# rdd0582/mri_superresolution

Hardware: AMD Instinct MI355X
Metric: 2D MRI slices/sec (train fwd+bwd) 256×256 U-Net; PSNR/SSIM vs ref (higher is better)
Workload: dtype bf16; 1 GPU; UNetSuperRes base_filters=64 depth=4, 256x256 slices -> 512x512, batch=16/GPU bf16, L1+SSIM(0.4), train step fwd+bwd+Adam+SSIM metric; global_batch=16, parallelism=dp1

## Files before the change

### include/mrisr.h

```cpp
#ifndef MRISR_H
#define MRISR_H

#include <stddef.h>
#include <stdint.h>

#ifdef __cplusplus
extern "C" {
#endif

#define MRISR_OK 0
#define MRISR_E_ARG (-1)
#define MRISR_E_SHAPE (-2)
#define MRISR_E_DTYPE (-3)
#define MRISR_E_HIP (-4)
#define MRISR_E_UNSUPPORTED (-5)

#define MRISR_F32 0
#define MRISR_BF16 1
#define MRISR_F16 2

#define MRISR_SRC_RAW 0
#define MRISR_SRC_NORM 1
#define MRISR_SRC_RELU 2
#define MRISR_SP_NONE 0
#define MRISR_SP_POOL2 1
#define MRISR_SP_UP2 2
#define MRISR_COMBINE_CONCAT 0
#define MRISR_COMBINE_BLEND 1
#ifndef MRISR_STAT_SLOTS
#define MRISR_STAT_SLOTS 16
#endif
#define MRISR_SP_HEAD 3
#define MRISR_OUT_PLAIN 0
#define MRISR_OUT_PIXEL_SHUFFLE2 1

typedef struct {
    const void* ptr;
    const float* scale;
    const float* shift;
    int32_t C, H, W;
    int32_t mode;
    int32_t spatial;
    int32_t off_y, off_x;
} mrisr_src;

typedef struct {
    int32_t dtype;
    int32_t N, H, W;
    int32_t Cin, Cout;
    int32_t ksize;
    int32_t nsrc;
    int32_t combine;
    int32_t out_mode;
    int32_t groups;
    int32_t relu_out;
    mrisr_src src[2];
    const float* blend_alpha;
    const void* wpacked;
    const float* bias;
    void* out;
    double* stats;
    const void* relu_mask;
    int32_t cu_limit;
    int32_t reserved_;
    const void* wpacked_ring;
} mrisr_conv_desc;

const char* mrisr_last_error(void);
int mrisr_version(void);
int mrisr_stat_slots(void);

size_t mrisr_packed_weight_bytes(int dtype, int Cout, int Cin, int ksize);
#define MRISR_PACK_RING 256
#define MRISR_PACK_UPADJ 512
int mrisr_conv_ring_bn(int dtype, int Cout, int Cin, int ksize);
size_t mrisr_packed_weight_bytes_ring(int dtype, int Cout, int Cin, int ksize);
int mrisr_pack_weights(int dtype, const float* w, int Cout, int Cin, int ksize, int transpose_flip,
                       void* packed, void* stream);
typedef struct {
    const float* w;
    void* packed;
    int32_t Cout, Cin, ksize, transpose_flip;
} mrisr_pack_job;
int mrisr_pack_weights_batched(int dtype, const mrisr_pack_job* jobs_device, int njobs, void* stream);
int mrisr_conv_forward(const mrisr_conv_desc* d, void* stream);
int mrisr_conv_variant(const mrisr_conv_desc* d, int wgrad, char* out, size_t n);
int mrisr_conv_wgrad(const mrisr_conv_desc* d, const void* dy, float* dw, float* workspace, size_t workspace_floats,
                     void* stream);
size_t mrisr_conv_wgrad_workspace_floats(const mrisr_conv_desc* d);

size_t mrisr_packed_weight_bytes_upadj(int dtype, int Cout, int Cin, int ksize);
int mrisr_conv_upadj(const mrisr_conv_desc* d, const void* g, void* d_low, void* stream);

int mrisr_stem_forward(int dtype, const float* x, const float* w, void* out, double* stats,
                       int N, int H, int W, int Cout, int groups, void* stream);
int mrisr_stem_wgrad(int dtype, const float* x, const void* dy, float* dw,
                     int N, int H, int W, int Cout, void* stream);
int mrisr_stem_forward_multi(int dtype, const float* x, const float* w, void* out, double* stats,
                             int N, int H, int W, int Cin, int Cout, int groups, void* stream);
int mrisr_stem_wgrad_multi(int dtype, const float* x, const void* dy, float* dw,
                           int N, int H, int W, int Cin, int Cout, void* stream);

int mrisr_gn_finalize(const double* stats, const float* gamma, const float* beta, float* scale,
                      float* shift, float* meanrstd, int N, int C, int groups, double count,
                      float eps, void* stream);

int mrisr_norm_pool2(int dtype, const void* x, const float* scale, const float* shift, void* out, int N,
                     int H, int W, int C, void* stream);
// ... 221 lines not shown
```

### mri_superresolution_amd/_lib.py

```python
from __future__ import annotations

import ctypes as C
import os

from .tuning import TUNING

_HERE = os.path.dirname(os.path.abspath(__file__))
LIB_PATH = TUNING.lib_path or os.path.join(_HERE, "libmrisr.so")

F32, BF16, F16 = 0, 1, 2
SRC_RAW, SRC_NORM, SRC_RELU = 0, 1, 2
SP_NONE, SP_POOL2, SP_UP2, SP_HEAD = 0, 1, 2, 3
COMBINE_CONCAT, COMBINE_BLEND = 0, 1
OUT_PLAIN, OUT_PIXEL_SHUFFLE2 = 0, 1
UP2_BILINEAR, UP2_BICUBIC, UP2_SHARP_BILINEAR = 0, 1, 2
WINDOW_F32, WINDOW_I16 = 0, 1
VOLBLEND_SET, VOLBLEND_ADD, VOLBLEND_FINISH = 0, 1, 2
MORPH_DILATE, MORPH_ERODE = 0, 1
RESAMPLE_LINEAR, RESAMPLE_CUBIC, RESAMPLE_AREA, RESAMPLE_LANCZOS4 = 1, 2, 3, 4
PACK_RING = 256
PACK_UPADJ = 512
STAT_SLOTS = 16

_vp, _fp, _dp, _i, _f, _d, _sz = C.c_void_p, C.c_void_p, C.c_void_p, C.c_int, C.c_float, C.c_double, C.c_size_t


class Src(C.Structure):
    _fields_ = [("ptr", _vp), ("scale", _fp), ("shift", _fp), ("C", C.c_int32), ("H", C.c_int32),
                ("W", C.c_int32), ("mode", C.c_int32), ("spatial", C.c_int32), ("off_y", C.c_int32),
                ("off_x", C.c_int32)]


class ConvDesc(C.Structure):
    _fields_ = [("dtype", C.c_int32), ("N", C.c_int32), ("H", C.c_int32), ("W", C.c_int32),
                ("Cin", C.c_int32), ("Cout", C.c_int32), ("ksize", C.c_int32), ("nsrc", C.c_int32),
                ("combine", C.c_int32), ("out_mode", C.c_int32), ("groups", C.c_int32),
                ("relu_out", C.c_int32), ("src", Src * 2), ("blend_alpha", _fp), ("wpacked", _vp),
                ("bias", _fp), ("out", _vp), ("stats", _dp), ("relu_mask", _vp), ("cu_limit", C.c_int32),
                ("reserved_", C.c_int32), ("wpacked_ring", _vp)]


class PackJob(C.Structure):
    _fields_ = [("w", _fp), ("packed", _vp), ("Cout", C.c_int32), ("Cin", C.c_int32), ("ksize", C.c_int32),
                ("transpose_flip", C.c_int32)]


class AugGeo(C.Structure):
    _fields_ = [("cos_a", C.c_float), ("sin_a", C.c_float), ("rotate", C.c_int32), ("flip", C.c_int32),
                ("fill", C.c_int32), ("brightness", C.c_float)]


class AugPhoto(C.Structure):
    _fields_ = [("contrast", C.c_float), ("mean", C.c_int32), ("noise_sigma", C.c_float), ("seed", C.c_uint32)]


class GnBwdFin(C.Structure):
    _fields_ = [("red", _fp), ("gamma", _fp), ("meanrstd", _fp), ("dgamma", _fp), ("dbeta", _fp),
                ("alpha_slots", _fp), ("alpha", _fp), ("dalpha", _fp), ("count", C.c_double),
                ("alpha_sign", C.c_float), ("groups", C.c_int32)]


class BlendBranch(C.Structure):
    _fields_ = [("x", _vp), ("scale", _fp), ("shift", _fp), ("meanrstd", _fp), ("red", _fp), ("alpha_slots", _fp),
                ("weight_mode", C.c_int32), ("reserved_", C.c_int32)]


class Consumer(C.Structure):
    _fields_ = [("da", _vp), ("C_total", C.c_int32), ("c_off", C.c_int32), ("H", C.c_int32),
                ("W", C.c_int32), ("spatial", C.c_int32), ("off_y", C.c_int32), ("off_x", C.c_int32),
                ("weight_mode", C.c_int32), ("head_out", _fp), ("head_w", _fp), ("head_part", _fp),
                ("head_dw", _fp), ("head_db", _fp)]


SIGNATURES = {
    "mrisr_last_error": (C.c_char_p, []),
    "mrisr_version": (_i, []),
    "mrisr_stat_slots": (_i, []),
    "mrisr_packed_weight_bytes": (_sz, [_i, _i, _i, _i]),
    "mrisr_conv_ring_bn": (_i, [_i, _i, _i, _i]),
    "mrisr_packed_weight_bytes_ring": (_sz, [_i, _i, _i, _i]),
    "mrisr_pack_weights": (_i, [_i, _fp, _i, _i, _i, _i, _vp, _vp]),
    "mrisr_pack_weights_batched": (_i, [_i, _vp, _i, _vp]),
    "mrisr_conv_forward": (_i, [C.POINTER(ConvDesc), _vp]),
    "mrisr_packed_weight_bytes_upadj": (_sz, [_i, _i, _i, _i]),
    "mrisr_conv_upadj": (_i, [C.POINTER(ConvDesc), _vp, _vp, _vp]),
    "mrisr_conv_variant": (_i, [C.POINTER(ConvDesc), _i, C.c_char_p, _sz]),
    "mrisr_conv_wgrad": (_i, [C.POINTER(ConvDesc), _vp, _fp, _fp, _sz, _vp]),
    "mrisr_conv_wgrad_workspace_floats": (_sz, [C.POINTER(ConvDesc)]),
    "mrisr_stem_forward": (_i, [_i, _fp, _fp, _vp, _dp, _i, _i, _i, _i, _i, _vp]),
    "mrisr_stem_wgrad": (_i, [_i, _fp, _vp, _fp, _i, _i, _i, _i, _vp]),
    "mrisr_stem_forward_multi": (_i, [_i, _fp, _fp, _vp, _dp, _i, _i, _i, _i, _i, _i, _vp]),
    "mrisr_stem_wgrad_multi": (_i, [_i, _fp, _vp, _fp, _i, _i, _i, _i, _i, _vp]),
    "mrisr_gn_finalize": (_i, [_dp, _fp, _fp, _fp, _fp, _fp, _i, _i, _i, _d, _f, _vp]),
    "mrisr_norm_pool2": (_i, [_i, _vp, _fp, _fp, _vp, _i, _i, _i, _i, _vp]),
    "mrisr_norm_upsample2": (_i, [_i, _vp, _fp, _fp, _vp, _i, _i, _i, _i, _vp]),
    "mrisr_norm_blend": (_i, [_i, _vp, _fp, _fp, _vp, _fp, _fp, _fp, _vp, _i, _i, _i, _i, _vp]),
    "mrisr_upsample2_stats": (_i, [_i, _vp, _vp, _dp, _i, _i, _i, _i, _i, _vp]),
    "mrisr_upsample2_adjoint": (_i, [_i, _vp, _vp, _i, _i, _i, _i, _vp]),
    "mrisr_act_bwd_reduce": (_i, [_i, _vp, _fp, _fp, _fp, _i, C.POINTER(Consumer), _fp, _vp, _fp, _fp, _i, _i, _i, _i, _i, _vp]),
    "mrisr_act_bwd_finalize": (_i, [_fp, _fp, _fp, _fp, _fp, _fp, _i, _i, _i, _d, _fp, _fp, _fp, _f, _vp]),
    "mrisr_act_bwd_apply": (_i, [_i, _vp, _vp, _fp, _vp, _i, _i, _i, _i, _i, _fp, _vp]),
    "mrisr_act_bwd_apply_fused": (_i, [_i, _vp, _fp, _fp, _i, C.POINTER(Consumer), _fp, _fp, C.POINTER(GnBwdFin), _vp, _i, _i,
                                       _i, _i, _vp]),
    "mrisr_act_bwd_onepass_slots": (_i, []),
    "mrisr_act_bwd_onepass_barrier_words": (_i, []),
    "mrisr_act_bwd_onepass_ok": (_i, [_i, _i, C.POINTER(Consumer), _i, _i, _i, _i]),
# ... 40 lines not shown
    "mrisr_resample_taps": (_i, [_i, _i, _i, _i, _vp, _vp, _fp]),
    "mrisr_f32_resample_letterbox": (_i, [_fp, _i, _i, _i, _vp, _fp, _i, _i, _vp, _fp, _i, _i, _i, _i, _i, _i, _f, _i, _fp, _vp, _vp]),
    "mrisr_f32_percentile_workspace_bytes": (_sz, [_i]),
    "mrisr_f32_percentile_bounds": (_i, [_fp, _sz, _i, _d, _d, _fp, _vp, _vp]),
    "mrisr_f32_window_normalise": (_i, [_fp, _fp, _sz, _i, _fp, _vp]),
    "mrisr_f32_window_restore": (_i, [_fp, _fp, _sz, _i, _i, _vp, _vp]),
    "mrisr_f32_volume_up2_blend": (_i, [_fp, _i, _i, _i, _i, _fp, _i, _i, _i, _vp, _vp]),
    "mrisr_f32_volume_down2": (_i, [_fp, _i, _i, _i, _i, _fp, _vp]),
    "mrisr_f32_volume_up2": (_i, [_fp, _i, _i, _i, _i, _i, _fp, _vp]),
    "mrisr_f32_volume_metrics": (_i, [_fp, _fp, _i, _i, _i, _f, _f, _i, _dp, _vp]),
    "mrisr_volume_metrics_finalize": (_i, [_dp, _i, _i, _i, _f, _dp, _vp]),
    "mrisr_f32_volume_metrics_masked": (_i, [_fp, _fp, _vp, _i, _i, _i, _f, _f, _i, _dp, _vp]),
    "mrisr_volume_metrics_finalize_masked": (_i, [_dp, _i, _i, _i, _f, _dp, _vp]),
    "mrisr_f32_volume_otsu_workspace_bytes": (_sz, []),
    "mrisr_f32_volume_otsu_mask": (_i, [_fp, _i, _i, _i, _vp, _dp, _vp, _vp]),
    "mrisr_u8_volume_morph": (_i, [_vp, _i, _i, _i, _i, _i, _vp, _vp, _vp]),
    "mrisr_u8_volume_label": (_i, [_vp, _i, _i, _i, _i, _i, _i, _vp, _vp]),
    "mrisr_u8_volume_label_workspace_bytes": (_sz, [_i, _i, _i]),
    "mrisr_u8_volume_keep_largest": (_i, [_vp, _i, _i, _i, _i, _vp, _dp, _vp, _vp]),
    "mrisr_u8_volume_fill_holes": (_i, [_vp, _i, _i, _i, _i, _vp, _dp, _vp, _vp]),
}

_lib = None
ABI_VERSION = 314


def load():
    global _lib
    if _lib is not None:
        return _lib
    if not os.path.exists(LIB_PATH):
        raise RuntimeError(
            f"{LIB_PATH} not found: the HIP kernel library is not built. Run "
            "`python -m mri_superresolution_amd.build` (needs hipcc); there is no CPU fallback.")
    lib = C.CDLL(LIB_PATH)
    missing = [name for name in SIGNATURES if not hasattr(lib, name)]
    if missing:
        raise RuntimeError(f"{LIB_PATH} lacks {len(missing)} symbol(s) of include/mrisr.h ({', '.join(missing[:4])}...): "
                           "header/library drift - rebuild with `python -m mri_superresolution_amd.build`")
    for name, (res, args) in SIGNATURES.items():
        fn = getattr(lib, name)
        fn.restype = res
        fn.argtypes = args
    if int(lib.mrisr_version()) != ABI_VERSION:
        raise RuntimeError(f"{LIB_PATH} is version {int(lib.mrisr_version())}, these bindings need {ABI_VERSION} (struct layouts "
                           "changed): rebuild with `python -m mri_superresolution_amd.build`")
    global STAT_SLOTS
# ... 48 lines not shown
```

### mri_superresolution_amd/csrc/api.cpp

```cpp
#include "common.h"
thread_local char g_mrisr_err[512] = "";
extern "C" const char* mrisr_last_error(void) { return g_mrisr_err; }
extern "C" int mrisr_version(void) { return 314; }
extern "C" int mrisr_stat_slots(void) { return MRISR_STAT_SLOTS; }
```

### mri_superresolution_amd/csrc/conv_common.h

```cpp
#pragma once
#include "common.h"

constexpr int kConvThreads = 256;
constexpr int kRowBytes = 64;
constexpr int kMaxHaloIter = 6;

__device__ __forceinline__ int swz(int row) { return (row >> 2) & 3; }
__device__ __forceinline__ int lds_off(int row, int chunk) {
    return row * kRowBytes + ((chunk ^ swz(row)) << 4);
}

constexpr int kHaloRowBytes = 80;
__device__ __forceinline__ int halo_off(int row, int chunk) { return row * kHaloRowBytes + (chunk << 4); }

static inline size_t conv_halo_bytes() { return (size_t)kMaxHaloIter * 64 * kHaloRowBytes; }
constexpr int kDmaHaloRows = 340;
constexpr int kDmaHaloBytes = kDmaHaloRows * 64;
static inline size_t conv_halo_total(bool dma) { return dma ? 4 * (size_t)kDmaHaloBytes : 2 * conv_halo_bytes(); }
static inline bool conv_weights_stationary(int nchunks, size_t wimg, bool dma = false) {
    return nchunks * wimg + conv_halo_total(dma) + (64 + 128) * sizeof(float) <= 159 * 1024;
}
static inline int conv_wgrad_fast(int dtype, int loader, int ks, int tw_log2, int Cout, int Cin) {
    if (dtype == MRISR_F32 || loader != MRISR_SP_NONE || ks != 3 || tw_log2 != 5) return 0;
    const int nfo = Cout % 64 == 0 ? 2 : (Cout <= 32 ? 1 : 0), nfi = Cin % 64 == 0 ? 2 : (Cin <= 32 ? 1 : 0);
// ... 30 lines not shown
    const float* shift;
    int C, H, W, mode, off_y, off_x;
    unsigned img_bytes;
};

struct ConvParams {
    SrcDev src[2];
    const float* blend_alpha;
    const void* wpacked;
    const float* bias;
    void* out;
    double* stats;
    const void* mask;
    const void* dy;
    float* dw;
    float* wsp;
    int N, H, W, Cin, CinP, Cout, CoutP;
    int nsrc, combine, out_mode, groups, relu_out;
    int tw_log2, th, tiles_x, tiles_y, ncb, nchunks;
    int ksplit;
    int ws;
    int ntiles, tiles_per_block;
    int cus;
    int dbg;
};
#ifdef MRISR_TUNING
#define DBG(p) ((p).dbg)
#else
#define DBG(p) 0
#endif

#define PIN_F(q, src, f) { auto v__ = (src).f; asm volatile("" : "+s"(v__)); (q).f = v__; }
__device__ __forceinline__ ConvParams pin_params(const ConvParams& in) {
    ConvParams q = in;
    PIN_F(q, in, H) PIN_F(q, in, W) PIN_F(q, in, Cout) PIN_F(q, in, N) PIN_F(q, in, nchunks) PIN_F(q, in, tw_log2)
    PIN_F(q, in, th) PIN_F(q, in, tiles_x) PIN_F(q, in, tiles_y) PIN_F(q, in, nsrc) PIN_F(q, in, dbg)
    PIN_F(q, in, groups) PIN_F(q, in, relu_out) PIN_F(q, in, out) PIN_F(q, in, stats) PIN_F(q, in, bias)
    PIN_F(q, in, dy) PIN_F(q, in, dw) PIN_F(q, in, wsp) PIN_F(q, in, mask) PIN_F(q, in, Cin) PIN_F(q, in, combine)
    PIN_F(q, in, src[0].ptr) PIN_F(q, in, src[0].scale) PIN_F(q, in, src[0].shift) PIN_F(q, in, src[0].C)
    PIN_F(q, in, src[0].H) PIN_F(q, in, src[0].W) PIN_F(q, in, src[0].mode) PIN_F(q, in, src[0].off_y)
    PIN_F(q, in, src[0].off_x) PIN_F(q, in, src[0].img_bytes)
    PIN_F(q, in, src[1].ptr) PIN_F(q, in, src[1].scale) PIN_F(q, in, src[1].shift) PIN_F(q, in, src[1].C)
    PIN_F(q, in, src[1].H) PIN_F(q, in, src[1].W) PIN_F(q, in, src[1].mode) PIN_F(q, in, src[1].off_y)
    PIN_F(q, in, src[1].off_x) PIN_F(q, in, src[1].img_bytes)
    return q;
}
// ... 258 lines not shown
```

### mri_superresolution_amd/csrc/conv_fwd.hip

```cpp
#include <stdlib.h>
#include <string.h>

#include "conv_common.h"

int num_cus();
int conv_fill_params(const mrisr_conv_desc* d, ConvParams& p, const char* who) {
    if (!d) MRISR_FAIL(MRISR_E_ARG, "%s: null descriptor", who);
    if (!mrisr_dtype_ok(d->dtype)) MRISR_FAIL(MRISR_E_DTYPE, "%s: dtype %d", who, d->dtype);
    if (d->ksize != 1 && d->ksize != 3) MRISR_FAIL(MRISR_E_UNSUPPORTED, "%s: ksize %d", who, d->ksize);
    if (d->nsrc < 1 || d->nsrc > 2) MRISR_FAIL(MRISR_E_ARG, "%s: nsrc %d", who, d->nsrc);
    if (d->N <= 0 || d->H <= 0 || d->W <= 0 || d->Cin <= 0 || d->Cout <= 0)
        MRISR_FAIL(MRISR_E_SHAPE, "%s: bad dims N%d H%d W%d Cin%d Cout%d", who, d->N, d->H, d->W, d->Cin, d->Cout);
    const int vec = mrisr_vec(d->dtype);
    memset(&p, 0, sizeof(p));
    int csum = 0;
    for (int s = 0; s < d->nsrc; ++s) {
        const mrisr_src& a = d->src[s];
        if (!a.ptr) MRISR_FAIL(MRISR_E_ARG, "%s: src%d null", who, s);
        if (a.C % vec) MRISR_FAIL(MRISR_E_SHAPE, "%s: src%d channels %d not a multiple of %d", who, s, a.C, vec);
        if (a.mode == MRISR_SRC_NORM && (!a.scale || !a.shift)) MRISR_FAIL(MRISR_E_ARG, "%s: src%d NORM without scale/shift", who, s);
        if (s > 0 && a.spatial != MRISR_SP_NONE) MRISR_FAIL(MRISR_E_UNSUPPORTED, "%s: spatial transform on src1", who);
        if (d->nsrc > 1 && a.spatial != MRISR_SP_NONE) MRISR_FAIL(MRISR_E_UNSUPPORTED, "%s: spatial transform with 2 sources", who);
        int vh = a.H, vw = a.W;
        if (a.spatial == MRISR_SP_POOL2) { vh = a.H / 2; vw = a.W / 2; }
// ... 84 lines not shown
        bool raw = true;
        for (int i = 0; i < d->nsrc; ++i) raw = raw && d->src[i].mode == MRISR_SRC_RAW;
        snprintf(out, n, "conv_wgrad_rows_kernel<%s,%d,%d,%d>", t, d->Cout % 64 ? 1 : 2, d->Cin % 64 ? 1 : 2, raw ? 1 : 0);
    } else if (wgrad) {
        snprintf(out, n, "conv_wgrad_kernel<%s,%d,%d,%d>", t, loader, d->ksize,
                 conv_wgrad_fast(d->dtype, loader, d->ksize, p.tw_log2, d->Cout, d->Cin));
    } else if (conv_ring_eligible(d, p)) {
        snprintf(out, n, "conv_ring_kernel<%s,2,4>", t);
    } else if (conv_pc_eligible(d, p)) {
        snprintf(out, n, "conv_pc_kernel<%s,%d%s>", t, d->src[0].mode == MRISR_SRC_NORM ? 1 : 0, conv_pc_kind(d, p) == 2 ? ",64" : "");
    } else if (conv1x1_gemm_eligible(d, p)) {
        snprintf(out, n, "conv1x1_gemm_kernel<%s,%d>", t, d->src[0].mode == MRISR_SRC_NORM ? 1 : 0);
    } else {
        const int BN = conv_choose_bn(d->Cout);
        const size_t wimg = (size_t)d->ksize * d->ksize * BN * kRowBytes;
        const bool dma = conv_dma_halo(p, d->src[0].spatial);
        const int ws = conv_weights_stationary(p.nchunks, wimg, dma) ? 1 : 0;
        snprintf(out, n, "conv_igemm_kernel<%s,%d,%d,%d,%d,%d,%d>", t, BN, loader, d->ksize, ws,
                 d->out_mode == MRISR_OUT_PIXEL_SHUFFLE2 ? 1 : (d->relu_mask ? kEpiMask : 0), dma ? 1 : 0);
    }
    return MRISR_OK;
}

extern "C" int mrisr_conv_forward(const mrisr_conv_desc* d, void* stream) {
    ConvParams p;
    int rc = conv_fill_params(d, p, "conv_forward");
    if (rc) return rc;
    if (!d->wpacked || !d->out) MRISR_FAIL(MRISR_E_ARG, "conv_forward: null weights/out");
    if (d->out_mode == MRISR_OUT_PIXEL_SHUFFLE2 && (d->Cout % 16)) MRISR_FAIL(MRISR_E_SHAPE, "conv_forward: pixel shuffle needs Cout%%16==0");
    if (d->relu_mask && (d->out_mode != MRISR_OUT_PLAIN || d->Cout % (mrisr_vec(d->dtype))))
        MRISR_FAIL(MRISR_E_UNSUPPORTED, "conv_forward: relu_mask needs a plain output with Cout a multiple of the 16-byte vector");
    if (d->stats && (d->groups <= 0 || d->Cout % d->groups)) MRISR_FAIL(MRISR_E_SHAPE, "conv_forward: Cout %d not divisible by groups %d", d->Cout, d->groups);
    if (conv_ring_eligible(d, p)) return launch_conv_ring(d, p, (hipStream_t)stream);
    if (conv_pc_eligible(d, p)) return launch_conv_pc(d, p, (hipStream_t)stream);
    if (conv1x1_gemm_eligible(d, p)) return launch_conv1x1_gemm(d, p, (hipStream_t)stream);
    if (d->ksize == 3 && d->W > 16 && d->H >= 16) {
        p.th = 16; p.tw_log2 = 4;
        p.tiles_x = ceil_div(d->W, 16); p.tiles_y = ceil_div(d->H, 16);
    }
    const int sp = d->src[0].spatial;
    hipStream_t s = (hipStream_t)stream;
    const int BN = conv_choose_bn(d->Cout);
    if (d->dtype == MRISR_BF16) return launch_conv_igemm_bf16(p, BN, sp, d->ksize, s);
    if (d->dtype == MRISR_F16) return launch_conv_igemm_f16(p, BN, sp, d->ksize, s);
    return launch_conv_igemm_f32(p, BN, sp, d->ksize, s);
}
```

### mri_superresolution_amd/csrc/conv_igemm.h

```cpp
#pragma once
#include <mutex>
#include <type_traits>

#include "conv_common.h"

template <typename T> struct Mma;
template <> struct Mma<bf16_t> {
    typedef bf16x8 frag;
    static __device__ __forceinline__ f32x16 run(frag a, frag b, f32x16 c) {
        return __builtin_amdgcn_mfma_f32_32x32x16_bf16(a, b, c, 0, 0, 0);
    }
};
template <> struct Mma<f16_t> {
    typedef f16x8 frag;
    static __device__ __forceinline__ f32x16 run(frag a, frag b, f32x16 c) {
        return __builtin_amdgcn_mfma_f32_32x32x16_f16(a, b, c, 0, 0, 0);
    }
};
template <> struct Mma<float> {
    typedef f32x4 frag;
    static __device__ __forceinline__ f32x16 run(frag a, frag b, f32x16 c) {
#pragma unroll
        for (int j = 0; j < 4; ++j) c = __builtin_amdgcn_mfma_f32_32x32x2f32(a[j], b[j], c, 0, 0, 0);
        return c;
// ... 685 lines not shown
                        [&](int st) { pace_dma(plan, st); });
                PT_MARK(6)
                if (it_jj == p.nchunks - 1) {
                    epilogue(it_n, it_ty0, it_tx0);
                    PT_MARK(4)
                    if (p.stats && (!nx_valid || nx_n != it_n)) flush_stats(it_n);
                    PT_MARK(9)
                }
            } else {
#pragma unroll
                for (int st = 0; st < 2 * NTAPS; ++st) pace_dma(plan, st);
            }
            gkc = nx_kc;
            it_jj = nx_jj; it_tile = nx_tile; it_n = nx_n; it_ty0 = nx_ty0; it_tx0 = nx_tx0;
        }
#ifdef MRISR_PHASE_TIMING
        if (blockIdx.x == gridDim.x / 2 && lane == 0) {
            pt_acc[10] = __builtin_amdgcn_s_memrealtime() - pt_r0;
#pragma unroll
            for (int k = 0; k < 12; ++k) atomicAdd(&g_phase_cycles[threadIdx.x >> 6][k], pt_acc[k]);
            if (threadIdx.x == 0) atomicAdd(&g_phase_cycles[0][11], 1ull);
        }
#endif
        return;
    }
    int cur_tile = tile0, cur_kc = 0, cur_n = 0, cur_ty0 = 0, cur_tx0 = 0;
    int nxt_tile = tile0, nxt_kc = 0, nxt_n = 0, nxt_ty0 = 0, nxt_tx0 = 0;
    int ep_n = 0, ep_ty0 = 0, ep_tx0 = 0;
    bool ep_pending = false;
    const int nitems0 = nh0 * p.nchunks;
    if (nitems > 0) {
        decode(cur_tile, cur_n, cur_ty0, cur_tx0);
        set_geom(cur_n, cur_ty0, cur_tx0);
        issue(cur_n, 0, cur_ty0, cur_tx0);
    }
    if constexpr (!WS) {
        if (half == 0 && nitems0 > 0) dma_weights(0, 0, std::integral_constant<int, 4>{});
        __builtin_amdgcn_s_waitcnt(0x0f70);
        if constexpr (NH != 1) __syncthreads();
    }
    if constexpr (NH == 1) {
        if (wave == 0 && nitems > 0) lds_aff[lane] = pf.aff;
        __syncthreads();
    }
    if (__builtin_amdgcn_readfirstlane(threadIdx.x) >= 256) __builtin_amdgcn_s_setprio(1);
    PT_DECL
// ... 40 lines not shown
                ep_pending = true;
                ep_n = cur_n; ep_ty0 = cur_ty0; ep_tx0 = cur_tx0;
            }
            cur_tile = nxt_tile; cur_kc = nxt_kc; cur_n = nxt_n; cur_ty0 = nxt_ty0; cur_tx0 = nxt_tx0;
            if constexpr (NH == 1) {
                if (wave == 0) lds_aff[lane] = pf.aff;
            }
          }
            PT_MARK(6)
        }
        if (!(DBG(p) & 64)) __syncthreads();
#ifdef MRISR_PHASE_TIMING
        if (phase >= 0 && (phase & 1) == 0) PT_MARK(5) else PT_MARK(7)
#endif
    }
#ifdef MRISR_PHASE_TIMING
    if (blockIdx.x == gridDim.x / 2 && lane == 0) {
        pt_acc[10] = __builtin_amdgcn_s_memrealtime() - pt_r0;
#pragma unroll
        for (int k = 0; k < 12; ++k) atomicAdd(&g_phase_cycles[threadIdx.x >> 6][k], pt_acc[k]);
        if (threadIdx.x == 0) atomicAdd(&g_phase_cycles[0][11], 1ull);
    }
#endif
}

#ifdef MRISR_PHASE_TIMING
static int conv_igemm_phase(unsigned long long* out96) {
    unsigned long long v[96] = {};
    if (!out96) return (int)hipMemcpyToSymbol(HIP_SYMBOL(g_phase_cycles), v, sizeof(v));
    const int rc = (int)hipMemcpyFromSymbol(v, HIP_SYMBOL(g_phase_cycles), sizeof(v));
    if (rc) return rc;
    for (int k = 0; k < 96; ++k) out96[k] += v[k];
    return 0;
}
#endif

int launch_gn_stats(int dtype, const void* x, double* stats, int N, int HW, int C, int groups, hipStream_t s);

template <typename T, int BN, int SPATIAL, int KS, bool DMA>
static int launch_conv_v(ConvParams& p, hipStream_t s) {
    const size_t wimg = (size_t)KS * KS * BN * kRowBytes;
    p.ws = conv_weights_stationary(p.nchunks, wimg, DMA) ? 1 : 0;
    const size_t lds = conv_halo_total(DMA) + (p.ws ? p.nchunks : 2) * wimg + (BN + 128) * sizeof(float);
    p.ntiles = p.N * p.tiles_y * p.tiles_x;
    int per_cb = p.cus / p.ncb;
    if (per_cb < 1) per_cb = 1;
// ... 71 lines not shown
```

### mri_superresolution_amd/csrc/norm.hip

```cpp
#include "common.h"

__global__ void gn_finalize_kernel(const double* __restrict__ stats, const float* __restrict__ gamma,
                                   const float* __restrict__ beta, float* __restrict__ scale,
                                   float* __restrict__ shift, float* __restrict__ meanrstd, int N, int C,
                                   int groups, double count, float eps) {
    const int idx = blockIdx.x * blockDim.x + threadIdx.x;
    if (idx >= N * C) return;
    const int n = idx / C, c = idx - n * C;
    const int gs = C / groups, g = c / gs;
    typedef __attribute__((ext_vector_type(2))) double f64x2;
    f64x2 v[MRISR_STAT_SLOTS];
#pragma unroll
    for (int k = 0; k < MRISR_STAT_SLOTS; ++k) v[k] = *reinterpret_cast<const f64x2*>(stats + ((size_t)(k * N + n) * groups + g) * 2);
    double s = 0.0, ss = 0.0;
#pragma unroll
    for (int k = 0; k < MRISR_STAT_SLOTS; ++k) { s += v[k][0]; ss += v[k][1]; }
    const double mean = s / count;
    double var = ss / count - mean * mean;
    if (var < 0) var = 0;
    const float rstd = (float)(1.0 / sqrt(var + (double)eps));
    const float m = (float)mean;
    const float sc = gamma[c] * rstd;
    scale[idx] = sc;
    shift[idx] = beta[c] - m * sc;
    if (c == g * gs) {
        meanrstd[((size_t)n * groups + g) * 2] = m;
        meanrstd[((size_t)n * groups + g) * 2 + 1] = rstd;
    }
}

extern "C" int mrisr_gn_finalize(const double* stats, const float* gamma, const float* beta, float* scale,
                                 float* shift, float* meanrstd, int N, int C, int groups, double count,
                                 float eps, void* stream) {
    if (!stats || !gamma || !beta || !scale || !shift || !meanrstd) MRISR_FAIL(MRISR_E_ARG, "gn_finalize: null pointer");
    if (groups <= 0 || C % groups) MRISR_FAIL(MRISR_E_SHAPE, "gn_finalize: C %d groups %d", C, groups);
    gn_finalize_kernel<<<ceil_div(N * C, 256), 256, 0, (hipStream_t)stream>>>(stats, gamma, beta, scale, shift,
                                                                             meanrstd, N, C, groups, count, eps);
    MRISR_CHECK_LAUNCH("gn_finalize");
    return MRISR_OK;
}

struct ConsumerDev {
    const void* da;
    int C_total, c_off, H, W, spatial, off_y, off_x, weight_mode;
    const float* head_out;
    const float* head_w;
    float* head_part;
    float* head_dw;
    float* head_db;
};
struct ActBwdParams {
// ... 1915 lines not shown
```

### mri_superresolution_amd/engine.py

```python
from __future__ import annotations

import ctypes as C
from dataclasses import dataclass
from typing import Dict, List, Optional, Tuple

import torch

from . import _lib as L
from .launch import GN_GROUPS, Consumer, dgrad_desc, gn_finalize, marshal_consumers
from .tuning import TUNING


def _dt(dtype: torch.dtype) -> int:
    if dtype == torch.bfloat16:
        return L.BF16
    if dtype == torch.float16:
        return L.F16
    if dtype == torch.float32:
        return L.F32
    raise ValueError(f"unsupported compute dtype {dtype} (use torch.float32, torch.float16 or torch.bfloat16)")


@dataclass(frozen=True, eq=False)
class Node:
    name: str
    C: int
    gamma: str
    beta: str
    shuffled: bool = False


@dataclass(frozen=True, eq=False)
# ... 117 lines not shown
        for j in range(1, depth):
            skip, cout = xs[depth - 1 - j], f * 2 ** (depth - 1 - j)
            up = node(f"up{j}.up.1", cout, f"up{j}.up.2.weight", f"up{j}.up.2.bias")
            self.layers.append(Layer(f"up{j}.up.1", 2 * cout, cout, 1, (Source(u),), up, post_up=True))
            u = dconv(f"up{j}.conv", (Source(skip), Source(up)), 2 * cout, cout)
        fb = node("final_up_bilinear.1", f // 2, "final_up_bilinear.2.weight", "final_up_bilinear.2.bias")
        self.layers.append(Layer("final_up_bilinear.1", f, f // 2, 3, (Source(u),), fb, up_src=True))
        ps = node("final_up_pixelshuffle.conv", f // 2, "final_up_pixelshuffle.norm.weight",
                  "final_up_pixelshuffle.norm.bias", shuffled=True)
        self.layers.append(Layer("final_up_pixelshuffle.conv", f, 2 * f, 3, (Source(u),), ps, bias=True,
                                 out_mode=L.OUT_PIXEL_SHUFFLE2))
        fc = node("final_conv.0", f // 2, "final_conv.1.weight", "final_conv.1.bias")
        self.layers.append(Layer("final_conv.0", f // 2, f // 2, 3, (Source(fb), Source(ps)), fc,
                                 combine=L.COMBINE_BLEND, blend_src=True))
        self.head_in = fc
        self._blend_sibling: Dict[Node, Node] = {}
        for layer in self.layers:
            if layer.combine == L.COMBINE_BLEND:
                a, b = (src.node for src in layer.srcs)
                self._blend_sibling[a], self._blend_sibling[b] = b, a
        self._packed: Dict[tuple, torch.Tensor] = {}
        self._packed_token = None
        self.timer: Optional[KernelTimer] = None

    def _launch(self, kind, desc, fn):
        if self.timer is None:
            return fn()
        flops = 2.0 * desc.N * desc.H * desc.W * desc.Cin * desc.Cout * desc.ksize * desc.ksize
        if kind == "upadj":
            flops /= 4
        buf = C.create_string_buffer(96)
        L.call("mrisr_conv_variant", C.byref(desc), {"wgrad": 1, "upadj": 2}.get(kind, 0), buf, 96)
        self.timer.launch(buf.value.decode(), flops, fn)

    def _packed_buf(self, layer: Layer, w, dt: int, flip: int, ring: bool = False, upadj: bool = False):
        key = (layer.name, dt, "upadj") if upadj else (layer.name, dt, flip, "ring") if ring else (layer.name, dt, flip)
        buf = self._packed.get(key)
        if buf is None or buf.device != w.device:
            if upadj:
                nbytes = L.load().mrisr_packed_weight_bytes_upadj(dt, layer.cout, layer.cin, layer.ks)
            else:
                size = L.load().mrisr_packed_weight_bytes_ring if ring else L.load().mrisr_packed_weight_bytes
                nbytes = size(dt, layer.cin if flip else layer.cout, layer.cout if flip else layer.cin, layer.ks)
            buf = torch.empty(nbytes, dtype=torch.uint8, device=w.device)
            self._packed[key] = buf
        return buf
# ... 73 lines not shown
        if s.spatial == L.SP_POOL2:
            return n.H // 2, n.W // 2
        if s.spatial == L.SP_UP2:
            return 2 * n.H, 2 * n.W
        return n.H, n.W

    def forward(self, params, x: torch.Tensor, dtype: torch.dtype, training: bool, weights_token=None):
        dt = _dt(dtype)
        dev = x.device
        N, _, H, W = x.shape
        es = 4 if dtype == torch.float32 else 2
        mins = 2 ** (self.depth - 1)
        if H < mins or W < mins:
            raise ValueError(f"input must be at least {mins}x{mins} ({self.depth - 1} 2x2 max-pools)")
        st = L.stream_ptr()
        f = self.f
        p = _Pass()
        p.x, p.dtype, p.N = x, dtype, N
        per = L.STAT_SLOTS * N * GN_GROUPS * 2
        p.arena = torch.zeros(len(self.nodes) * per, dtype=torch.float64, device=dev)
        ns = p.nodes = {n: _NodeState(p.arena[i * per:(i + 1) * per]) for i, n in enumerate(self.nodes.values())}
        p.layers = {}

        def finalize(n: Node):
            o = ns[n]
            o.scale, o.shift, o.meanrstd = gn_finalize(o.stats, params[n.gamma], params[n.beta], N, n.C, o.H, o.W, st)

        if training or weights_token is None or self._packed_token != (dt, weights_token):
            self._pack_all(params, dt, st, weights_token)
        s = ns[self.stem]
        s.H, s.W = H, W
        s.raw = torch.empty((N, H, W, f), dtype=dtype, device=dev)
        L.call("mrisr_stem_forward_multi", dt, x.data_ptr(), params["inc.double_conv.0.weight"].data_ptr(),
               s.raw.data_ptr(), s.stats.data_ptr(), N, H, W, self.cin, f, GN_GROUPS, st,
               nbytes=N * H * W * (4 * self.cin + f * es))
        finalize(self.stem)

        for layer in self.layers:
            sn = ns[layer.srcs[0].node]
            sC = layer.srcs[0].node.C
            vh, vw = self._virtual_hw(layer.srcs[0], sn)
            aux = None
            if layer.pool_src:
                vh, vw = sn.H // 2, sn.W // 2
                aux = torch.empty((N, vh, vw, sC), dtype=dtype, device=dev)
                L.call("mrisr_norm_pool2", dt, sn.raw.data_ptr(), sn.scale.data_ptr(), sn.shift.data_ptr(),
                       aux.data_ptr(), N, sn.H, sn.W, sC, st, nbytes=N * sn.H * sn.W * sC * es * 1.25)
            if layer.up_src:
                vh, vw = 2 * sn.H, 2 * sn.W
                aux = torch.empty((N, vh, vw, sC), dtype=dtype, device=dev)
                L.call("mrisr_norm_upsample2", dt, sn.raw.data_ptr(), sn.scale.data_ptr(), sn.shift.data_ptr(),
                       aux.data_ptr(), N, sn.H, sn.W, sC, st, nbytes=N * sn.H * sn.W * sC * es * 5)
            fused_blend = (layer.blend_src and not training and es == 2 and layer.cout == 32
                           and (layer.name, dt, 0, "ring") in self._packed)
            if layer.blend_src and not fused_blend:
                a, b = sn, ns[layer.srcs[1].node]
                if (a.H, a.W, sC) != (b.H, b.W, layer.srcs[1].node.C):
                    raise RuntimeError(f"{layer.name}: blend sources differ in shape")
                aux = torch.empty((N, a.H, a.W, sC), dtype=dtype, device=dev)
                L.call("mrisr_norm_blend", dt, a.raw.data_ptr(), a.scale.data_ptr(), a.shift.data_ptr(), b.raw.data_ptr(),
                       b.scale.data_ptr(), b.shift.data_ptr(), params["alpha"].data_ptr(), aux.data_ptr(),
                       N, a.H, a.W, sC, st, nbytes=N * a.H * a.W * sC * es * 3)
            offs = []
            for src in layer.srcs:
                h, w = (vh, vw) if (layer.pool_src or layer.up_src) else self._virtual_hw(src, ns[src.node])
                dy, dx = vh - h, vw - w
                if dy < 0 or dx < 0:
                    raise RuntimeError(f"{layer.name}: source larger than the conv input")
                offs.append((dy // 2, dx // 2))
            p.layers[layer] = _LayerState(vh, vw, offs, aux)
            o, oC = ns[layer.out], layer.out.C
            if layer.out_mode == L.OUT_PIXEL_SHUFFLE2 or layer.post_up:
                o.H, o.W = 2 * vh, 2 * vw
            else:
                o.H, o.W = vh, vw
            o.raw = torch.empty((N, o.H, o.W, oC), dtype=dtype, device=dev)
            d = self._desc(layer, p, dt, params, fused_blend)
            d.wpacked = self._packed[(layer.name, dt, 0)].data_ptr()
            d.wpacked_ring = L.ptr(self._packed.get((layer.name, dt, 0, "ring")))
            d.bias = params[layer.name + ".bias"].data_ptr() if layer.bias else None
            if layer.post_up:
                zlow = torch.empty((N, vh, vw, oC), dtype=dtype, device=dev)
                d.out, d.stats = zlow.data_ptr(), None
            else:
                d.out, d.stats = o.raw.data_ptr(), o.stats.data_ptr()
            self._launch("fwd", d, lambda: L.call("mrisr_conv_forward", C.byref(d), st))
            if layer.post_up:
                L.call("mrisr_upsample2_stats", dt, zlow.data_ptr(), o.raw.data_ptr(), o.stats.data_ptr(),
                       N, vh, vw, oC, GN_GROUPS, st, nbytes=N * vh * vw * oC * es * 5)
            finalize(layer.out)

        hn, hC = ns[self.head_in], self.head_in.C
        p.out = torch.empty((N, self.cout, hn.H, hn.W), dtype=torch.float32, device=dev)
        L.call("mrisr_head_forward_multi", dt, hn.raw.data_ptr(), hn.scale.data_ptr(), hn.shift.data_ptr(),
               params["final_conv.3.weight"].data_ptr(), params["final_conv.3.bias"].data_ptr(), p.out.data_ptr(),
               N, hn.H, hn.W, hC, self.cout, st, nbytes=N * hn.H * hn.W * (hC * es + 4 * self.cout))
        return p.out, (p if training else None)

    def backward(self, params, grads, ctx: _Pass, dout: torch.Tensor, bucket_hook=None):
        dtype = ctx.dtype
        dt = _dt(dtype)
        es = 4 if dtype == torch.float32 else 2
        N = ctx.N
        x = ctx.x
        dev = x.device
        st = L.stream_ptr()
        ns, ls = ctx.nodes, ctx.layers
        dout = dout.contiguous()

        narr = N * L.load().mrisr_act_bwd_onepass_barrier_words()
        SL = L.load().mrisr_act_bwd_onepass_slots() if es == 2 else 1
        red_sizes = [SL * N * n.C * 2 + 256 + narr + (N * (n.C + 1) if n is self.head_in else 0) for n in self.nodes.values()]
        red_arena = torch.zeros(sum(red_sizes), dtype=torch.float32, device=dev)
# ... 240 lines not shown
```

### mri_superresolution_amd/launch.py

```python
from __future__ import annotations

from dataclasses import dataclass
from typing import Optional, Sequence, Tuple

import torch

from . import _lib as L

GN_GROUPS, GN_EPS = 8, 1e-5


@dataclass
class Consumer:
    da: torch.Tensor
    C_total: int
    c_off: int
    H: int
    W: int
    spatial: int
    off_y: int
    off_x: int
    weight_mode: int = 0
    head: Optional[Tuple[torch.Tensor, ...]] = None

# ... 4 lines not shown
    cons = (L.Consumer * 2)()
    for c, k in zip(cons, consumers):
        c.da = k.da.data_ptr()
        c.C_total, c.c_off, c.H, c.W = k.C_total, k.c_off, k.H, k.W
        c.spatial, c.off_y, c.off_x, c.weight_mode = k.spatial, k.off_y, k.off_x, k.weight_mode
        if k.head is not None:
            c.head_out, c.head_w, c.head_part, c.head_dw, c.head_db = (t.data_ptr() for t in k.head)
    return cons


def dgrad_desc(dt: int, dy: torch.Tensor, Cin: int, Cout: int, ks: int, wpacked: torch.Tensor, out: torch.Tensor,
               wpacked_ring: Optional[torch.Tensor] = None, cu_limit: int = 0) -> L.ConvDesc:
    N, H, W, _ = dy.shape
    d = L.ConvDesc()
    d.dtype, d.N, d.H, d.W = dt, N, H, W
    d.Cin, d.Cout, d.ksize, d.nsrc = Cout, Cin, ks, 1
    d.combine, d.out_mode, d.groups, d.relu_out = L.COMBINE_CONCAT, L.OUT_PLAIN, 0, 0
    s = d.src[0]
    s.ptr, s.C, s.H, s.W, s.mode, s.spatial = dy.data_ptr(), Cout, H, W, L.SRC_RAW, L.SP_NONE
    d.wpacked, d.wpacked_ring, d.out, d.cu_limit = wpacked.data_ptr(), L.ptr(wpacked_ring), out.data_ptr(), cu_limit
    return d


def gn_finalize(stats: torch.Tensor, gamma: torch.Tensor, beta: torch.Tensor, N: int, Cc: int, H: int, W: int, stream):
    dev = stats.device
    scale = torch.empty(N * Cc, dtype=torch.float32, device=dev)
    shift = torch.empty(N * Cc, dtype=torch.float32, device=dev)
    meanrstd = torch.empty(N * GN_GROUPS * 2, dtype=torch.float32, device=dev)
    L.call("mrisr_gn_finalize", stats.data_ptr(), gamma.data_ptr(), beta.data_ptr(), scale.data_ptr(), shift.data_ptr(),
           meanrstd.data_ptr(), N, Cc, GN_GROUPS, float((Cc // GN_GROUPS) * H * W), GN_EPS, stream)
    return scale, shift, meanrstd
```

Measured before the change: 2082 slices/s.

## Fuse GroupNorm finalize into conv forward via last-block arrival counter

Adds a last-block-done pattern to the implicit-GEMM conv forward kernel. Each block atomically increments a sharded arrival counter, and the final block to arrive computes GroupNorm mean/rstd and per-channel scale/shift from the accumulated stats, then resets the counter. This removes a separate gn_finalize kernel launch per eligible layer on the bf16/f16 path. In exchange every block pays an extra vmcnt wait, two barriers and atomics, the tail block does serial finalize work, and ring, pc and 1x1-gemm variants are excluded.

```diff
diff --git a/include/mrisr.h b/include/mrisr.h
--- a/include/mrisr.h
+++ b/include/mrisr.h
@@ -43,6 +43,19 @@
     int32_t spatial;
     int32_t off_y, off_x;
 } mrisr_src;
+
+#define MRISR_GN_FIN_WORDS 1040
+typedef struct {
+    const float* gamma;
+    const float* beta;
+    float* scale;
+    float* shift;
+    float* meanrstd;
+    uint32_t* counter;
+    double count;
+    float eps;
+    int32_t C;
+} mrisr_gn_fin;
 
 typedef struct {
     int32_t dtype;
@@ -64,6 +77,7 @@
     int32_t cu_limit;
     int32_t reserved_;
     const void* wpacked_ring;
+    mrisr_gn_fin fin;
 } mrisr_conv_desc;
 
 const char* mrisr_last_error(void);
@@ -84,6 +98,8 @@
 } mrisr_pack_job;
 int mrisr_pack_weights_batched(int dtype, const mrisr_pack_job* jobs_device, int njobs, void* stream);
 int mrisr_conv_forward(const mrisr_conv_desc* d, void* stream);
+int mrisr_conv_fuses_finalize(const mrisr_conv_desc* d);
+int mrisr_gn_fin_ok(int dtype, int N, int C, int groups);
 int mrisr_conv_variant(const mrisr_conv_desc* d, int wgrad, char* out, size_t n);
 int mrisr_conv_wgrad(const mrisr_conv_desc* d, const void* dy, float* dw, float* workspace, size_t workspace_floats,
                      void* stream);
diff --git a/mri_superresolution_amd/_lib.py b/mri_superresolution_amd/_lib.py
--- a/mri_superresolution_amd/_lib.py
+++ b/mri_superresolution_amd/_lib.py
@@ -31,13 +31,21 @@
                 ("off_x", C.c_int32)]
 
 
+class GnFin(C.Structure):
+    _fields_ = [("gamma", _fp), ("beta", _fp), ("scale", _fp), ("shift", _fp), ("meanrstd", _fp), ("counter", _vp),
+                ("count", C.c_double), ("eps", C.c_float), ("C", C.c_int32)]
+
+
+GN_FIN_WORDS = 1040
+
+
 class ConvDesc(C.Structure):
     _fields_ = [("dtype", C.c_int32), ("N", C.c_int32), ("H", C.c_int32), ("W", C.c_int32),
                 ("Cin", C.c_int32), ("Cout", C.c_int32), ("ksize", C.c_int32), ("nsrc", C.c_int32),
                 ("combine", C.c_int32), ("out_mode", C.c_int32), ("groups", C.c_int32),
                 ("relu_out", C.c_int32), ("src", Src * 2), ("blend_alpha", _fp), ("wpacked", _vp),
                 ("bias", _fp), ("out", _vp), ("stats", _dp), ("relu_mask", _vp), ("cu_limit", C.c_int32),
-                ("reserved_", C.c_int32), ("wpacked_ring", _vp)]
+                ("reserved_", C.c_int32), ("wpacked_ring", _vp), ("fin", GnFin)]
 
 
 class PackJob(C.Structure):
@@ -82,6 +90,8 @@
     "mrisr_pack_weights": (_i, [_i, _fp, _i, _i, _i, _i, _vp, _vp]),
     "mrisr_pack_weights_batched": (_i, [_i, _vp, _i, _vp]),
     "mrisr_conv_forward": (_i, [C.POINTER(ConvDesc), _vp]),
+    "mrisr_conv_fuses_finalize": (_i, [C.POINTER(ConvDesc)]),
+    "mrisr_gn_fin_ok": (_i, [_i, _i, _i, _i]),
     "mrisr_packed_weight_bytes_upadj": (_sz, [_i, _i, _i, _i]),
     "mrisr_conv_upadj": (_i, [C.POINTER(ConvDesc), _vp, _vp, _vp]),
     "mrisr_conv_variant": (_i, [C.POINTER(ConvDesc), _i, C.c_char_p, _sz]),
@@ -168,7 +178,7 @@
 }
 
 _lib = None
-ABI_VERSION = 314
+ABI_VERSION = 315
 
 
 def load():
diff --git a/mri_superresolution_amd/csrc/api.cpp b/mri_superresolution_amd/csrc/api.cpp
--- a/mri_superresolution_amd/csrc/api.cpp
+++ b/mri_superresolution_amd/csrc/api.cpp
@@ -1,5 +1,5 @@
 #include "common.h"
 thread_local char g_mrisr_err[512] = "";
 extern "C" const char* mrisr_last_error(void) { return g_mrisr_err; }
-extern "C" int mrisr_version(void) { return 314; }
+extern "C" int mrisr_version(void) { return 315; }
 extern "C" int mrisr_stat_slots(void) { return MRISR_STAT_SLOTS; }
diff --git a/mri_superresolution_amd/csrc/conv_common.h b/mri_superresolution_amd/csrc/conv_common.h
--- a/mri_superresolution_amd/csrc/conv_common.h
+++ b/mri_superresolution_amd/csrc/conv_common.h
@@ -1,5 +1,6 @@
 #pragma once
 #include "common.h"
+#include "gn_finalize.h"
 
 constexpr int kConvThreads = 256;
 constexpr int kRowBytes = 64;
@@ -76,6 +77,7 @@
     int ws;
     int ntiles, tiles_per_block;
     int cus;
+    GnFinDev fin;
     int dbg;
 };
 #ifdef MRISR_TUNING
diff --git a/mri_superresolution_amd/csrc/conv_fwd.hip b/mri_superresolution_amd/csrc/conv_fwd.hip
--- a/mri_superresolution_amd/csrc/conv_fwd.hip
+++ b/mri_superresolution_amd/csrc/conv_fwd.hip
@@ -130,10 +130,25 @@
     return MRISR_OK;
 }
 
+static bool conv_fuses_finalize(const mrisr_conv_desc* d, const ConvParams& p) {
+    if (!gn_fin_requested(d->fin) || !d->stats || d->groups <= 0 || d->Cout % d->groups) return false;
+    const int C = d->out_mode == MRISR_OUT_PIXEL_SHUFFLE2 ? d->Cout / 4 : d->Cout;
+    if (!gn_fin_complete(d->fin) || d->fin.C != C || !mrisr_gn_fin_ok(d->dtype, d->N, C, d->groups)) return false;
+    if (conv_ring_eligible(d, p) || conv_pc_eligible(d, p) || conv1x1_gemm_eligible(d, p)) return false;
+    return ((d->Cout / d->groups) & 3) == 0;
+}
+
+extern "C" int mrisr_conv_fuses_finalize(const mrisr_conv_desc* d) {
+    ConvParams p;
+    if (conv_fill_params(d, p, "conv_fuses_finalize")) return 0;
+    return conv_fuses_finalize(d, p) ? 1 : 0;
+}
+
 extern "C" int mrisr_conv_forward(const mrisr_conv_desc* d, void* stream) {
     ConvParams p;
     int rc = conv_fill_params(d, p, "conv_forward");
     if (rc) return rc;
+    if (conv_fuses_finalize(d, p)) p.fin = gn_fin_dev(d->fin);
     if (!d->wpacked || !d->out) MRISR_FAIL(MRISR_E_ARG, "conv_forward: null weights/out");
     if (d->out_mode == MRISR_OUT_PIXEL_SHUFFLE2 && (d->Cout % 16)) MRISR_FAIL(MRISR_E_SHAPE, "conv_forward: pixel shuffle needs Cout%%16==0");
     if (d->relu_mask && (d->out_mode != MRISR_OUT_PLAIN || d->Cout % (mrisr_vec(d->dtype))))
diff --git a/mri_superresolution_amd/csrc/conv_igemm.h b/mri_superresolution_amd/csrc/conv_igemm.h
--- a/mri_superresolution_amd/csrc/conv_igemm.h
+++ b/mri_superresolution_amd/csrc/conv_igemm.h
@@ -731,6 +731,8 @@
             if (threadIdx.x == 0) atomicAdd(&g_phase_cycles[0][11], 1ull);
         }
 #endif
+        if (has_stats && p_in.fin.counter)
+        gn_fin_block(p_in.fin, p.stats, p.N, p.groups, blockIdx.x, gridDim.x, reinterpret_cast<unsigned*>(smem));
         return;
     }
     int cur_tile = tile0, cur_kc = 0, cur_n = 0, cur_ty0 = 0, cur_tx0 = 0;
@@ -817,6 +819,8 @@
         if (threadIdx.x == 0) atomicAdd(&g_phase_cycles[0][11], 1ull);
     }
 #endif
+    if (has_stats && p_in.fin.counter)
+        gn_fin_block(p_in.fin, p.stats, p.N, p.groups, blockIdx.x, gridDim.x, reinterpret_cast<unsigned*>(smem));
 }
 
 #ifdef MRISR_PHASE_TIMING
diff --git a/mri_superresolution_amd/csrc/gn_finalize.h b/mri_superresolution_amd/csrc/gn_finalize.h
--- /dev/null
+++ b/mri_superresolution_amd/csrc/gn_finalize.h
@@ -0,0 +1,99 @@
+#pragma once
+#include "common.h"
+
+struct GnFinDev {
+    const float* gamma;
+    const float* beta;
+    float* scale;
+    float* shift;
+    float* meanrstd;
+    unsigned* counter;
+    double count;
+    float eps;
+    int C;
+};
+
+constexpr int kGnFinMaxPairs = 1024;
+constexpr int kGnFinMaxC = 2048;
+static inline bool gn_fin_shape_ok(int N, int C, int groups) {
+    return N > 0 && groups > 0 && C > 0 && C % groups == 0 && C <= kGnFinMaxC && (long)N * groups <= kGnFinMaxPairs;
+}
+static inline GnFinDev gn_fin_dev(const mrisr_gn_fin& f) {
+    return GnFinDev{f.gamma, f.beta, f.scale, f.shift, f.meanrstd, f.counter, f.count, f.eps, f.C};
+}
+static inline bool gn_fin_requested(const mrisr_gn_fin& f) { return f.counter != nullptr; }
+static inline bool gn_fin_complete(const mrisr_gn_fin& f) {
+    return f.gamma && f.beta && f.scale && f.shift && f.meanrstd && f.counter && f.C > 0 && f.count > 0;
+}
+
+__device__ __forceinline__ void gn_mean_rstd(double s, double ss, double count, float eps, float& m, float& rstd) {
+    const double mean = s / count;
+    double var = ss / count - mean * mean;
+    if (var < 0) var = 0;
+    rstd = (float)(1.0 / sqrt(var + (double)eps));
+    m = (float)mean;
+}
+__device__ __forceinline__ void gn_affine(float gamma, float beta, float m, float rstd, float& sc, float& sh) {
+    sc = gamma * rstd;
+    sh = beta - m * sc;
+}
+
+constexpr int kGnFinGroups = MRISR_GN_FIN_WORDS / 16 - 1;
+__device__ __forceinline__ unsigned gn_fin_ngroups(unsigned n) { return n <= 256u ? 16u : (unsigned)kGnFinGroups; }
+__device__ __forceinline__ bool gn_fin_arrive(unsigned* ctr, unsigned id, unsigned n) {
+    const unsigned G = gn_fin_ngroups(n), g = id % G;
+    const unsigned ngroups = min(n, G), members = (n - g + G - 1) / G;
+    if (__hip_atomic_fetch_add(ctr + g * 16, 1u, __ATOMIC_RELAXED, __HIP_MEMORY_SCOPE_AGENT) + 1 != members) return false;
+    return __hip_atomic_fetch_add(ctr + kGnFinGroups * 16, 1u, __ATOMIC_RELAXED, __HIP_MEMORY_SCOPE_AGENT) + 1 == ngroups;
+}
+__device__ __forceinline__ void gn_fin_reset(unsigned* ctr, int lane) {
+    for (int k = lane; k <= kGnFinGroups; k += 64) __hip_atomic_store(ctr + k * 16, 0u, __ATOMIC_RELAXED, __HIP_MEMORY_SCOPE_AGENT);
+}
+
+template <int P>
+__device__ __forceinline__ void gn_finalize_pairs(const GnFinDev& f, const double* stats, int N, int groups, int p0, int lane) {
+    static_assert(P > 0 && P <= 64, "one lane per pair");
+    const int npairs = N * groups, gs = f.C / groups;
+    const int cnt = min(P, npairs - p0);
+    float m = 0.f, rstd = 0.f;
+    if (lane < cnt) {
+        const GLOBAL_AS double* sp = (const GLOBAL_AS double*)stats + (size_t)(p0 + lane) * 2;
+        double v[MRISR_STAT_SLOTS][2];
+#pragma unroll
+        for (int k = 0; k < MRISR_STAT_SLOTS; ++k) {
+            v[k][0] = __hip_atomic_load(sp + (size_t)k * npairs * 2, __ATOMIC_RELAXED, __HIP_MEMORY_SCOPE_AGENT);
+            v[k][1] = __hip_atomic_load(sp + (size_t)k * npairs * 2 + 1, __ATOMIC_RELAXED, __HIP_MEMORY_SCOPE_AGENT);
+        }
+        double s = 0.0, ss = 0.0;
+#pragma unroll
+        for (int k = 0; k < MRISR_STAT_SLOTS; ++k) { s += v[k][0]; ss += v[k][1]; }
+        gn_mean_rstd(s, ss, f.count, f.eps, m, rstd);
+        f.meanrstd[(size_t)(p0 + lane) * 2] = m;
+        f.meanrstd[(size_t)(p0 + lane) * 2 + 1] = rstd;
+    }
+    const int nel = cnt * gs;
+    for (int e0 = 0; e0 < nel; e0 += 64) {
+        const int e = e0 + lane, src = min(e / gs, P - 1);
+        const float pm = __shfl(m, src, 64), pr = __shfl(rstd, src, 64);
+        if (e < nel) {
+            const int idx = p0 * gs + e, c = idx % f.C;
+            float sc, sh;
+            gn_affine(f.gamma[c], f.beta[c], pm, pr, sc, sh);
+            f.scale[idx] = sc;
+            f.shift[idx] = sh;
+        }
+    }
+}
+
+__device__ __forceinline__ void gn_fin_block(const GnFinDev& f, const double* stats, int N, int groups, unsigned block,
+                                             unsigned nblocks, unsigned* flag) {
+    asm volatile("s_waitcnt vmcnt(0)" ::: "memory");
+    __syncthreads();
+    if (threadIdx.x == 0) *flag = gn_fin_arrive(f.counter, block, nblocks) ? 1u : 0u;
+    __syncthreads();
+    if (*flag == 0u) return;
+    constexpr int P = 16;
+    const int wave = threadIdx.x >> 6, lane = threadIdx.x & 63, nwaves = blockDim.x >> 6;
+    for (int p0 = wave * P; p0 < N * groups; p0 += nwaves * P) gn_finalize_pairs<P>(f, stats, N, groups, p0, lane);
+    if (wave == 0) gn_fin_reset(f.counter, lane);
+}
diff --git a/mri_superresolution_amd/csrc/norm.hip b/mri_superresolution_amd/csrc/norm.hip
--- a/mri_superresolution_amd/csrc/norm.hip
+++ b/mri_superresolution_amd/csrc/norm.hip
@@ -1,4 +1,5 @@
 #include "common.h"
+#include "gn_finalize.h"
 
 __global__ void gn_finalize_kernel(const double* __restrict__ stats, const float* __restrict__ gamma,
                                    const float* __restrict__ beta, float* __restrict__ scale,
@@ -15,18 +16,19 @@
     double s = 0.0, ss = 0.0;
 #pragma unroll
     for (int k = 0; k < MRISR_STAT_SLOTS; ++k) { s += v[k][0]; ss += v[k][1]; }
-    const double mean = s / count;
-    double var = ss / count - mean * mean;
-    if (var < 0) var = 0;
-    const float rstd = (float)(1.0 / sqrt(var + (double)eps));
-    const float m = (float)mean;
-    const float sc = gamma[c] * rstd;
+    float m, rstd, sc, sh;
+    gn_mean_rstd(s, ss, count, eps, m, rstd);
+    gn_affine(gamma[c], beta[c], m, rstd, sc, sh);
     scale[idx] = sc;
-    shift[idx] = beta[c] - m * sc;
+    shift[idx] = sh;
     if (c == g * gs) {
         meanrstd[((size_t)n * groups + g) * 2] = m;
         meanrstd[((size_t)n * groups + g) * 2 + 1] = rstd;
     }
+}
+
+extern "C" int mrisr_gn_fin_ok(int dtype, int N, int C, int groups) {
+    return (dtype == MRISR_BF16 || dtype == MRISR_F16) && gn_fin_shape_ok(N, C, groups) ? 1 : 0;
 }
 
 extern "C" int mrisr_gn_finalize(const double* stats, const float* gamma, const float* beta, float* scale,
diff --git a/mri_superresolution_amd/engine.py b/mri_superresolution_amd/engine.py
--- a/mri_superresolution_amd/engine.py
+++ b/mri_superresolution_amd/engine.py
@@ -7,7 +7,7 @@
 import torch
 
 from . import _lib as L
-from .launch import GN_GROUPS, Consumer, dgrad_desc, gn_finalize, marshal_consumers
+from .launch import GN_GROUPS, Consumer, dgrad_desc, gn_fin_request, gn_finalize, gn_outputs, marshal_consumers
 from .tuning import TUNING
 
 
@@ -171,6 +171,8 @@
         self._packed: Dict[tuple, torch.Tensor] = {}
         self._packed_token = None
         self.timer: Optional[KernelTimer] = None
+        self.fused_finalize = True
+        self._fin_counters: Optional[torch.Tensor] = None
 
     def _launch(self, kind, desc, fn):
         if self.timer is None:
@@ -290,9 +292,26 @@
         ns = p.nodes = {n: _NodeState(p.arena[i * per:(i + 1) * per]) for i, n in enumerate(self.nodes.values())}
         p.layers = {}
 
-        def finalize(n: Node):
+        ctr = None
+        if self.fused_finalize and es == 2:
+            if self._fin_counters is None or self._fin_counters.device != dev:
+                self._fin_counters = torch.zeros(len(self.nodes) * L.GN_FIN_WORDS, dtype=torch.int32, device=dev)
+            ctr = self._fin_counters
+        node_index = {n: i for i, n in enumerate(self.nodes.values())}
+
+        def fin_request(n: Node) -> Optional[L.GnFin]:
             o = ns[n]
-            o.scale, o.shift, o.meanrstd = gn_finalize(o.stats, params[n.gamma], params[n.beta], N, n.C, o.H, o.W, st)
+            o.scale, o.shift, o.meanrstd = gn_outputs(N, n.C, dev)
+            if ctr is None or not L.load().mrisr_gn_fin_ok(dt, N, n.C, GN_GROUPS):
+                return None
+            i = node_index[n]
+            return gn_fin_request((o.scale, o.shift, o.meanrstd), params[n.gamma], params[n.beta],
+                                  ctr[i * L.GN_FIN_WORDS:(i + 1) * L.GN_FIN_WORDS], n.C, o.H, o.W)
+
+        def finalize(n: Node, fused: bool):
+            if not fused:
+                o = ns[n]
+                gn_finalize(o.stats, params[n.gamma], params[n.beta], N, n.C, o.H, o.W, st, out=(o.scale, o.shift, o.meanrstd))
 
         if training or weights_token is None or self._packed_token != (dt, weights_token):
             self._pack_all(params, dt, st, weights_token)
@@ -302,7 +321,8 @@
         L.call("mrisr_stem_forward_multi", dt, x.data_ptr(), params["inc.double_conv.0.weight"].data_ptr(),
                s.raw.data_ptr(), s.stats.data_ptr(), N, H, W, self.cin, f, GN_GROUPS, st,
                nbytes=N * H * W * (4 * self.cin + f * es))
-        finalize(self.stem)
+        fin_request(self.stem)
+        finalize(self.stem, False)
 
         for layer in self.layers:
             sn = ns[layer.srcs[0].node]
@@ -347,16 +367,21 @@
             d.wpacked = self._packed[(layer.name, dt, 0)].data_ptr()
             d.wpacked_ring = L.ptr(self._packed.get((layer.name, dt, 0, "ring")))
             d.bias = params[layer.name + ".bias"].data_ptr() if layer.bias else None
+            fin = fin_request(layer.out)
+            fused = fin is not None and not layer.post_up
             if layer.post_up:
                 zlow = torch.empty((N, vh, vw, oC), dtype=dtype, device=dev)
                 d.out, d.stats = zlow.data_ptr(), None
             else:
                 d.out, d.stats = o.raw.data_ptr(), o.stats.data_ptr()
+                if fused:
+                    d.fin = fin
+                    fused = bool(L.load().mrisr_conv_fuses_finalize(C.byref(d)))
             self._launch("fwd", d, lambda: L.call("mrisr_conv_forward", C.byref(d), st))
             if layer.post_up:
                 L.call("mrisr_upsample2_stats", dt, zlow.data_ptr(), o.raw.data_ptr(), o.stats.data_ptr(),
                        N, vh, vw, oC, GN_GROUPS, st, nbytes=N * vh * vw * oC * es * 5)
-            finalize(layer.out)
+            finalize(layer.out, fused)
 
         hn, hC = ns[self.head_in], self.head_in.C
         p.out = torch.empty((N, self.cout, hn.H, hn.W), dtype=torch.float32, device=dev)
diff --git a/mri_superresolution_amd/launch.py b/mri_superresolution_amd/launch.py
--- a/mri_superresolution_amd/launch.py
+++ b/mri_superresolution_amd/launch.py
@@ -50,11 +50,25 @@
     return d
 
 
-def gn_finalize(stats: torch.Tensor, gamma: torch.Tensor, beta: torch.Tensor, N: int, Cc: int, H: int, W: int, stream):
-    dev = stats.device
-    scale = torch.empty(N * Cc, dtype=torch.float32, device=dev)
-    shift = torch.empty(N * Cc, dtype=torch.float32, device=dev)
-    meanrstd = torch.empty(N * GN_GROUPS * 2, dtype=torch.float32, device=dev)
+def gn_outputs(N: int, Cc: int, dev):
+    return (torch.empty(N * Cc, dtype=torch.float32, device=dev), torch.empty(N * Cc, dtype=torch.float32, device=dev),
+            torch.empty(N * GN_GROUPS * 2, dtype=torch.float32, device=dev))
+
+
+def gn_count(Cc: int, H: int, W: int) -> float:
+    return float((Cc // GN_GROUPS) * H * W)
+
+
+def gn_fin_request(out, gamma: torch.Tensor, beta: torch.Tensor, counter: torch.Tensor, Cc: int, H: int, W: int) -> L.GnFin:
+    f = L.GnFin()
+    f.gamma, f.beta = gamma.data_ptr(), beta.data_ptr()
+    f.scale, f.shift, f.meanrstd = (t.data_ptr() for t in out)
+    f.counter, f.count, f.eps, f.C = counter.data_ptr(), gn_count(Cc, H, W), GN_EPS, Cc
+    return f
+
+
+def gn_finalize(stats: torch.Tensor, gamma: torch.Tensor, beta: torch.Tensor, N: int, Cc: int, H: int, W: int, stream, out=None):
+    scale, shift, meanrstd = out if out is not None else gn_outputs(N, Cc, stats.device)
     L.call("mrisr_gn_finalize", stats.data_ptr(), gamma.data_ptr(), beta.data_ptr(), scale.data_ptr(), shift.data_ptr(),
-           meanrstd.data_ptr(), N, Cc, GN_GROUPS, float((Cc // GN_GROUPS) * H * W), GN_EPS, stream)
+           meanrstd.data_ptr(), N, Cc, GN_GROUPS, gn_count(Cc, H, W), GN_EPS, stream)
     return scale, shift, meanrstd
```

New measurement: 2079 slices/s. No clear change (-0.1%).
